# sc15i2gp/daily-ray-trace

Hardware: AMD Instinct MI355X
Metric: Mpaths/s (pixels*spp/s) Cornell 1024^2 depth 8; achieved HBM GB/s % of peak (higher is better)
Workload: dtype f64

## Files before the change

### daily-ray-trace_amd/csrc/drt_kernels.h

```cpp
#pragma once

#include "drt_device.h"
#include "drt_build_rule.h"
#include <type_traits>
#include "../../include/drt_hip.h"


enum
{
    SF_PX = 0, SF_PY, SF_PZ, SF_RADIUS,
    SF_NX, SF_NY, SF_NZ,
    SF_UNX, SF_UNY, SF_UNZ,
    SF_VNX, SF_VNY, SF_VNZ,
    SF_ULEN, SF_VLEN,
    SF_COUNT
};
enum
{
    LF_PX = 0, LF_PY, LF_PZ, LF_RADIUS,
    LF_UX, LF_UY, LF_UZ,
    LF_VX, LF_VY, LF_VZ,
    LF_PDF,
    LF_COUNT
};

enum
{
    NEED_GLOSSY = 1u,
    NEED_EQR    = 2u,
    NEED_EQT    = 4u,
    NEED_CT     = 8u
};

struct BvhNode
{
    float   lo[2][3], hi[2][3];
// ... 877 lines not shown
#define DRT_TRACE_CONST 2
#endif
#if DRT_TRACE_CONST == 1
#define TRACE_CONST_BYTES ((sizeof(TraceConst) + 127u) & ~(size_t)127u)
#else
#define TRACE_CONST_BYTES ((size_t)0)
#endif
__device__ __forceinline__ uint32_t pinned_scalar(uint32_t v)
{
    asm volatile("" : "+s"(v));
    return v;
}
__device__ __forceinline__ const TraceConst &trace_const(const double *lds)
{
#if DRT_TRACE_CONST == 2
    uint32_t off = 0;
    asm volatile("" : "+s"(off));
    return *(const TraceConst *)((const char *)__builtin_amdgcn_kernarg_segment_ptr() + off);
#else
    uint32_t off = 0;
    asm volatile("" : "+v"(off));
    return *(const TraceConst *)((const char *)lds + off);
#endif
}
#define TRACE_LANE_ROWS 2u
#define TRACE_LW_BLK 0u
#define TRACE_LW_DRAWS 1u
#define TRACE_LW_SCANS 128u
#define TRACE_LW_SHADED 129u
__device__ __forceinline__ void lane_word_add(uint32_t *w, uint32_t v)
{
    (void)__hip_atomic_fetch_add(w, v, __ATOMIC_RELAXED, __HIP_MEMORY_SCOPE_WAVEFRONT);
}
#define DRT_TRACE_TAIL_MAX 8u
#ifndef DRT_TRACE_WAVES_PER_SIMD
#define DRT_TRACE_WAVES_PER_SIMD 3
#endif


#ifdef DRT_BRANCH_STATS
#define DRT_BS_WORDS 20
__device__ unsigned long long drt_branch_stats[DRT_BS_WORDS];
__device__ unsigned int drt_branch_waves_done;
#endif

template <bool SCENE_IN_LDS, bool TAIL, bool LIST, bool RAYS>
__device__ __forceinline__ void trace_paths(DevScene k_sc, DevCamera k_cam, TraceParams k_tp,
                                            uint64_t *records, uint64_t *headers,
                                            int32_t *k_hits, unsigned long long *k_counters,
                                            unsigned long long *k_work_counter, const DevRayTable &k_rt)
{
    extern __shared__ double lds_raw[];
#if DRT_TRACE_CONST == 1
    if (threadIdx.x == 0)
    {
        TraceConst *c = (TraceConst *)lds_raw;
        c->sc = k_sc;
        c->cam = k_cam;
        c->tp = k_tp;
        c->hits = k_hits;
        c->counters = k_counters;
        c->work_counter = k_work_counter;
    }
#endif
#if DRT_TRACE_CONST == 0
    const TraceConst k_all = {k_sc, k_cam, k_tp, records, headers, k_hits, k_counters, k_work_counter};
#define LC k_all
#else
#define LC trace_const(lds_raw)
#endif
#if DRT_TRACE_CONST == 2
#define LC_RT (((const TraceRaysConst &)trace_const(lds_raw)).rt)
#else
#define LC_RT k_rt
#endif
    SceneView sv;
    double *l_spd_tail = nullptr, *tail_state = nullptr;
    double *lane_area = nullptr;
    uint32_t *lane_words = nullptr;
    uint32_t TR, max_depth, vertex_words, block_words;
    bool tail_on, record_hits;
    {
    const DevScene &sc = k_sc;
    const TraceParams &tp = k_tp;
    sv.n_surf = sc.n_surf;
    sv.n_lights = sc.n_lights;
    if (SCENE_IN_LDS)
    {
        double *l_rows = lds_raw + TRACE_CONST_BYTES / 8;
        double *l_surf = l_rows + (size_t)SR_STRIDE * sc.n_surf;
        for (uint32_t k = threadIdx.x; k < SR_STRIDE * sc.n_surf; k += TRACE_BLOCK)
        {
            const uint32_t i = k / SR_STRIDE, f = k % SR_STRIDE;
            l_rows[k] = f < SF_COUNT ? sc.surf[f * sc.n_surf + i] : f == SR_TYPE ? __longlong_as_double((long long)sc.surf_type[i]) : 0.0;
        }
        double *l_lights = l_surf + (size_t)SF_COUNT * sc.n_surf;
        uint32_t *l_u32 = (uint32_t *)(l_lights + (size_t)LF_COUNT * sc.n_lights);
        uint32_t n_u32 = 2 * sc.n_surf + 2 * sc.n_lights;
        DevMaterial *l_mats = (DevMaterial *)((char *)l_u32 + (((size_t)n_u32 * 4 + 7) & ~(size_t)7));
        for (uint32_t k = threadIdx.x; k < SF_COUNT * sc.n_surf; k += TRACE_BLOCK) l_surf[k] = sc.surf[k];
        for (uint32_t k = threadIdx.x; k < LF_COUNT * sc.n_lights; k += TRACE_BLOCK) l_lights[k] = sc.lights[k];
        for (uint32_t k = threadIdx.x; k < sc.n_surf; k += TRACE_BLOCK)
        {
            l_u32[k] = sc.surf_type[k];
            l_u32[sc.n_surf + k] = sc.surf_mat[k];
        }
        for (uint32_t k = threadIdx.x; k < sc.n_lights; k += TRACE_BLOCK)
        {
            l_u32[2 * sc.n_surf + k] = sc.light_type[k];
            l_u32[2 * sc.n_surf + sc.n_lights + k] = sc.light_mat[k];
        }
// ... 5 lines not shown
        sv.lights = l_lights;
        sv.surf_type = l_u32;
        sv.surf_mat = l_u32 + sc.n_surf;
        sv.light_type = l_u32 + 2 * sc.n_surf;
        sv.light_mat = l_u32 + 2 * sc.n_surf + sc.n_lights;
        sv.mats = l_mats;
        sv.rows = l_rows;
        sv.bvh_nodes = nullptr;
        sv.bvh_leaf = nullptr;
    }
    else
    {
        sv.surf = sc.surf;
        sv.lights = sc.lights;
        sv.surf_type = sc.surf_type;
        sv.surf_mat = sc.surf_mat;
        sv.light_type = sc.light_type;
        sv.light_mat = sc.light_mat;
        sv.mats = sc.mats;
        sv.bvh_nodes = sc.bvh_nodes;
        sv.bvh_leaf = sc.bvh_leaf;
        __syncthreads();
    }

    TR = tp.tail_count;
    tail_on = TAIL && SCENE_IN_LDS && tp.tail_stage != nullptr;
    lane_area = SCENE_IN_LDS ? (double *)(sv.mats + sc.n_mat) : lds_raw + TRACE_CONST_BYTES / 8;
    if (tail_on)
    {
        l_spd_tail = lane_area;
        for (uint32_t k = threadIdx.x; k < tp.n_spd * TR; k += TRACE_BLOCK) l_spd_tail[k] = tp.spd_tail[k];
        lane_area += (size_t)tp.n_spd * TR;
    }
    lane_area += (size_t)(threadIdx.x >> 6) * ((TRACE_LANE_ROWS + (tail_on ? 1u + 2u * TR : 0u)) * 64u) + (threadIdx.x & 63u);
    lane_words = (uint32_t *)lane_area;
    lane_words[TRACE_LW_BLK] = 0u;
    lane_words[TRACE_LW_DRAWS] = 0u;
    lane_words[TRACE_LW_SCANS] = 0u;
    lane_words[TRACE_LW_SHADED] = 0u;
    if (tail_on)
    {
        tail_state = lane_area + (TRACE_LANE_ROWS + 1u) * 64u;
        __syncthreads();
    }
    max_depth = tp.max_depth;
    vertex_words = tp.vertex_words;
    block_words = tp.block_words;
    record_hits = tp.record_hits != 0u;
    if (*tp.overflow) return;
    }
    bool tail_ok = false;
    const uint32_t lane = threadIdx.x & 63u;
    uint64_t chunk_next = 0, chunk_end = 0;
    PathPos chunk_pos = {0, 0};

    uint32_t w_paths = 0;
#ifdef DRT_BRANCH_STATS
    uint64_t bs[DRT_BS_WORDS] = {};
#endif

    bool alive = false;
    bool exhausted = false;
    uint64_t rs = 1, hit_row = 0;
    uint32_t depth = 0, shaded = 0;
    uint32_t vis0_mask = 0;
    uint32_t plastic_mask = 0;
    V3 ro = v3(0, 0, 0), rd = v3(0, 0, 0);
    uint64_t *hdr = nullptr;
    uint32_t tbl = 0;
    uint32_t spare = ~0u, spare_tbl = ~0u;
    WavePool wp = {0u, 0u, 0u, 0u};

    for (;;)
    {
        unsigned long long idle_mask = __ballot(!alive);
        if (idle_mask != 0ull && !exhausted)
        {
            uint32_t want = (uint32_t)__popcll(idle_mask);
            uint32_t rank = (uint32_t)__popcll(idle_mask & ((1ull << lane) - 1ull));
            uint64_t avail = chunk_end - chunk_next;
            const uint32_t n_samples = LC.tp.n_samples;
            PathPos from = chunk_pos;
            uint32_t ahead = rank;
            if (avail < want)
            {
                if (!alive && rank < avail) alive = true;
                uint32_t taken = (uint32_t)avail;
                const TraceConst &c = LC;
                const uint64_t CHUNK = c.tp.chunk, n_paths_all = c.tp.n_paths;
                unsigned long long base = 0;
                if (lane == 0) base = atomicAdd(c.work_counter, (unsigned long long)CHUNK);
                base = __shfl(base, 0);
                if (base >= n_paths_all)
                {
                    exhausted = true;
                    chunk_next = chunk_end = 0;
                }
                else
                {
                    chunk_next = base;
                    chunk_end = (base + CHUNK < n_paths_all) ? base + CHUNK : n_paths_all;
                    chunk_pos = path_pos_of_id(base, n_samples);
                    uint64_t avail2 = chunk_end - chunk_next;
                    if (!alive && rank >= taken && (uint64_t)(rank - taken) < avail2)
                    {
                        alive = true;
                        from = chunk_pos;
                        ahead = rank - taken;
                    }
                    uint32_t used = (want - taken < avail2) ? (want - taken) : (uint32_t)avail2;
                    chunk_next += used;
                    chunk_pos = path_pos_step(chunk_pos, used, n_samples);
                }
            }
            else
            {
                if (!alive) alive = true;
                chunk_next += want;
                chunk_pos = path_pos_step(chunk_pos, want, n_samples);
            }
            bool started = alive && ((idle_mask >> lane) & 1ull);
            w_paths += (uint32_t)__popcll(__ballot(started));
            if (started)
            {
                const TraceConst &c = LC;
                const PathPos me = path_pos_step(from, ahead, n_samples);
                const uint64_t q = me.q;
                const uint64_t s_local = me.s;
                if (record_hits) hit_row = s_local * c.tp.n_pix + q;
                const uint64_t t = LIST ? (uint64_t)c.tp.pixel_list[q] : q;
                uint32_t i, j;
                tile_pixel_ij(t, c.tp.tile_w, i, j);
                uint32_t x = c.tp.x0 + i;
                uint32_t y = c.tp.y0 + j * c.tp.row_stride;
                uint32_t sample = c.tp.first_sample + (uint32_t)s_local;
                if (LIST) sample += c.tp.sample_base[t];
                uint64_t key = c.tp.seed + (((uint64_t)sample * (uint64_t)c.tp.height + (uint64_t)y) * (uint64_t)c.tp.width + (uint64_t)x);
                rs = drt_splitmix64(key);
                double weight = 1.0;
                if (RAYS) weight = table_ray(LC_RT, c.tp.width, t, x, y, sample, ro, rd);
                else
                {
                    uint32_t drawn = 0;
                    camera_ray(c.cam, c.tp.pixel_scheme, x, y, rs, drawn, ro, rd);
                    lane_word_add(lane_words + TRACE_LW_DRAWS, drawn);
                }
                depth = 0;
                shaded = 0;
                plastic_mask = 0;
                vis0_mask = 0;
                tail_ok = tail_on;
                if (tail_on)
                {
                    const uint32_t tr = pinned_scalar(TR);
#pragma unroll
                    for (uint32_t j = 0; j < DRT_TRACE_TAIL_MAX; j += 1)
                    {
                        if (j >= tr) break;
                        tail_state[(2u * j) * 64u] = 1.0;
                        tail_state[(2u * j + 1u) * 64u] = 0.0;
                    }
                }
                uint64_t slot = q * (uint64_t)c.tp.batch + s_local;
                hdr = headers + slot * REC_HEADER_WORDS;
                const double vignette = (RAYS ? weight : v_dot(rd, c.cam.forward)) * 1.0;
                hdr[1] = (uint64_t)__double_as_longlong(vignette);
                if (tail_on) lane_area[TRACE_LANE_ROWS * 64u] = vignette;
                if (record_hits)
                {
                    int32_t *h = c.hits + ((uint64_t)c.tp.hits_sample_offset * c.tp.n_pix + hit_row) * max_depth;
                    for (uint32_t d = 0; d < max_depth; d += 1) h[d] = -2;
                }
            }
        }
        if (!__any(alive)) break;

        if (!path_spare_block(LC.tp, wp, alive, shaded, spare, spare_tbl, lane))
        {
            hdr[0] = (uint64_t)HDR_TERM_NOT_DONE << 16;
            alive = false;
            lane_word_add(lane_words + TRACE_LW_SCANS, depth);
            lane_word_add(lane_words + TRACE_LW_SHADED, shaded);
        }
        if (alive)
        {
            TraceHit ip;
            find_ray_intersection<SCENE_IN_LDS>(sv, LC.sc, ip, ro, rd DRT_SCAN_STATS_ARG(bs + 16));
            if (record_hits)
            {
                const TraceConst &c = LC;
                c.hits[((uint64_t)c.tp.hits_sample_offset * c.tp.n_pix + hit_row) * max_depth + depth] = ip.index;
            }
            const DevMaterial &mat = sv.mats[ip.surface_mat];
            bool terminal = false;
            uint32_t term = 0, term_spd = 0;
            if (mat.is_black_body && !mat.is_emissive) terminal = true;
            else if (mat.is_black_body && mat.is_emissive)
            {
                terminal = true;
                term = 1;
                term_spd = (uint32_t)mat.emission_spd;
            }
            else
            {
                uint32_t blk = lane_words[TRACE_LW_BLK];
                path_open_vertex(LC.tp, wp, records, shaded, hdr, blk, tbl, spare, spare_tbl);
                lane_words[TRACE_LW_BLK] = blk;
                uint64_t *vrec = records + (uint64_t)blk * block_words + (uint64_t)(shaded & (REC_BLOCK_VERTICES - 1u)) * vertex_words;
// ... 217 lines not shown
                alive = false;
                lane_word_add(lane_words + TRACE_LW_SCANS, depth);
                lane_word_add(lane_words + TRACE_LW_SHADED, shaded);
            }
        }
    }

    uint64_t scans = lane_words[TRACE_LW_SCANS], n_shaded = lane_words[TRACE_LW_SHADED], draws = lane_words[TRACE_LW_DRAWS];
    uint64_t held = (uint64_t)(spare != ~0u) + (uint64_t)(spare_tbl != ~0u);
    for (int off = 32; off > 0; off >>= 1)
    {
        scans += __shfl_down(scans, off);
        n_shaded += __shfl_down(n_shaded, off);
        draws += __shfl_down(draws, off);
        held += __shfl_down(held, off);
    }
    uint64_t vals[6] = {w_paths, scans, n_shaded, n_shaded * sv.n_lights, draws, (uint64_t)wp.handed - held};
    unsigned long long *counters = LC.counters;
    for (int k = 0; k < 6; k += 1)
        if (lane == 0 && vals[k]) atomicAdd(&counters[k], (unsigned long long)vals[k]);
#ifdef DRT_BRANCH_STATS
    for (int k = 0; k < DRT_BS_WORDS; k += 1)
    {
        uint64_t v = bs[k];
        for (int off = 32; off > 0; off >>= 1) v += __shfl_down(v, off);
        if (lane == 0 && v) atomicAdd(&drt_branch_stats[k], (unsigned long long)v);
    }
    __threadfence();
    if (lane == 0 && atomicAdd(&drt_branch_waves_done, 1u) + 1u == gridDim.x * (TRACE_BLOCK / 64u))
    {
        unsigned long long t[DRT_BS_WORDS];
        for (int k = 0; k < DRT_BS_WORDS; k += 1) t[k] = atomicExch(&drt_branch_stats[k], 0ull);
        printf("DRT_BRANCH_STATS iters %llu lanes %llu | disc %llu %llu | ggx %llu %llu | coin %llu %llu | spec %llu %llu | all4 %llu | "
               "loop %llu again %llu | half %llu eqt %llu | uniform %llu | closest plane steps %llu skipped %llu | shadow plane steps %llu skipped %llu\n",
               t[0], t[1], t[2], t[3], t[4], t[5], t[6], t[7], t[8], t[9], t[10], t[11], t[12], t[13], t[14], t[15], t[16], t[17], t[18], t[19]);
        drt_branch_waves_done = 0u;
    }
#endif
#undef LC
#undef LC_RT
}

template <bool SCENE_IN_LDS, bool TAIL = false, bool LIST = false>
__global__ __launch_bounds__(TRACE_BLOCK, DRT_TRACE_WAVES_PER_SIMD) void drt_trace_kernel(DevScene k_sc, DevCamera k_cam, TraceParams k_tp,
                                                                 uint64_t *__restrict__ records, uint64_t *__restrict__ headers,
                                                                 int32_t *__restrict__ k_hits, unsigned long long *__restrict__ k_counters,
                                                                 unsigned long long *__restrict__ k_work_counter)
{
    const DevRayTable no_table = {nullptr, nullptr, nullptr, 0u, 0u, 0u, 0u};
    trace_paths<SCENE_IN_LDS, TAIL, LIST, false>(k_sc, k_cam, k_tp, records, headers, k_hits, k_counters, k_work_counter, no_table);
}

template <bool SCENE_IN_LDS, bool TAIL = false, bool LIST = false>
__global__ __launch_bounds__(TRACE_BLOCK, DRT_TRACE_WAVES_PER_SIMD) void drt_trace_rays_kernel(DevScene k_sc, DevCamera k_cam, TraceParams k_tp,
                                                                 uint64_t *__restrict__ records, uint64_t *__restrict__ headers,
                                                                 int32_t *__restrict__ k_hits, unsigned long long *__restrict__ k_counters,
                                                                 unsigned long long *__restrict__ k_work_counter, DevRayTable k_rt)
{
    trace_paths<SCENE_IN_LDS, TAIL, LIST, true>(k_sc, k_cam, k_tp, records, headers, k_hits, k_counters, k_work_counter, k_rt);
}


#define SHADE_BLOCK 256
#ifndef DRT_SHADE_WAVES_PER_SIMD
#define DRT_SHADE_WAVES_PER_SIMD 4
#endif
#define SHADE_WAVES (SHADE_BLOCK / 64)
#ifndef DRT_SHADE_WAVES_MULTISET
#define DRT_SHADE_WAVES_MULTISET(n) ((n) == 2 ? 3 : 2)
#endif
#define SHADE_WAVES_PER_SIMD_FOR(n) ((n) == 1 ? DRT_SHADE_WAVES_PER_SIMD : DRT_SHADE_WAVES_MULTISET(n))
#ifndef DRT_SHADE_WAVES_SIMPLE
#define DRT_SHADE_WAVES_SIMPLE 5
#endif
#define SHADE_MAX_SETS 4

struct ShadeParams
// ... 1411 lines not shown
```

### daily-ray-trace_amd/csrc/drt_launcher.hip

```cpp
#include "drt_kernels.h"
#include "drt_bvh_kernels.h"
#include "drt_adaptive_kernels.h"
#include "drt_sample_map_kernels.h"
#include "drt_denoise_kernels.h"
#include "drt_feature_kernels.h"
#include "drt_matte_kernels.h"
#include "drt_ray_kernels.h"
#include "drt_update_kernels.h"
#include "drt_build_kernels.h"
#include "drt_material_kernels.h"
#include "drt_depth_kernels.h"
#include "drt_window_kernels.h"
#include "drt_window_rule.h"
#include "drt_owned.h"

#include <algorithm>
#include <cmath>
#include <cstdarg>
#include <cstdio>
#include <cstdlib>
#include <cstring>
#include <map>
#include <string>
#include <chrono>
// ... 74 lines not shown
    DevBuf<double> d_tail_resume;
    uint32_t  batch_spp = 1;
    uint32_t  vertex_words = 0, vertex_shift = 0, block_words = 0;
    uint64_t  pool_blocks = 0;
    uint32_t  worst_blocks_per_path = 0;
    double    est_blocks_per_path = 0.0;
    struct Batch { uint32_t first_sample, n_samples; uint64_t seq; uint32_t row0, rows, hits_sample_offset, stride; const uint32_t *list; uint64_t list_len; };
    std::vector<Batch> inflight;
    uint64_t  next_seq = 1;
    uint64_t  redone_batches = 0, pool_peak = 0;
    DevBuf<int32_t> d_hits;
    uint64_t  hits_capacity = 0;
    uint32_t  hits_samples = 0;
    DevBuf<unsigned long long> d_counters;
    DevBuf<PrimaryHit> d_primary;
    DevBuf<uint64_t> d_queue;
    bool        bvh_pipeline = false;
    int         primary_grid_cap = 0, bounce_grid_cap = 0;
    DevBuf<double> d_xyz;
    DevBuf<uint8_t> d_bgra;
    bool      trace_tail = false;
    bool      tail_all_staged = false;
    bool      tail_resume = false;
    bool      dark_skip = true;
    bool      dark_skip_win = true;
    bool      no_fixed_lists = false;
    bool      simple_bdsfs = false;
    bool      no_closed_shade = false;
    bool      closed_lists = false;
    const double *d_spd_tail = nullptr;

    bool   scene_in_lds = true, spds_in_lds = true, use_bvh = false;
    size_t trace_lds = 0, shade_lds = 0;
    int    trace_grid_cap = 0, shade_grid_cap = 0;
    uint32_t trace_chunk_override = 0, shade_subs_override = ~0u, tail_period_override = 0;
    uint32_t shade_sets = 1, tail_first = 0, tail_count = 0;
    uint64_t n_pix = 0;

    std::vector<Event> ev;
    std::vector<double> ev_paths;
    size_t ev_used = 0;
    double trace_ms = 0.0, shade_ms = 0.0;
    uint64_t timed_pairs = 0;
    double min_sample_ms = 0.0, max_sample_ms = 0.0, avg_sample_ms = 0.0;

    bool film_used = false, adaptive_done = false;
    DevBuf<uint32_t> d_counts;
    DevBuf<uint32_t> d_alist[2];
    DevBuf<unsigned long long> d_keep;
    DevBuf<uint32_t> d_bkeep;
    DevBuf<uint32_t> d_ainfo;
    PinnedBuf<uint32_t> h_active;
    uint64_t film_gen = 0;
    uint64_t dn_gen = 0;
    bool     dn_valid = false;
    DevBuf<double> d_dn_mean, d_dn_var, d_dn_guide, d_dn_weights, d_dn_wsum;
    DevBuf<uint32_t> d_dn_unusable;
    uint32_t dn_window_cap = 0;
    std::vector<drt_material> ft_mats;
    std::vector<double> ft_spds;
    uint32_t ft_n_spd = 0, ft_S = 0;
    DevBuf<double> d_ft_mean, d_ft_m2, d_ft_colour;
    DevBuf<int32_t> d_ft_ids;
    DevBuf<uint32_t> d_ft_counts, d_ft_report;
    DevBuf<unsigned long long> d_ft_info;
    Event    ft_ev[2];
// ... 919 lines not shown
    const uint32_t deepest = (params->max_depth + REC_BLOCK_VERTICES - 1) / REC_BLOCK_VERTICES;
    ctx->worst_blocks_per_path = deepest + (deepest > REC_HEADER_BLOCKS ? 1u : 0u);
    if (deepest > REC_HEADER_BLOCKS + 2 * ctx->block_words)
        return fail(-2, "max_depth %u: a path's table block holds %u blocks beyond the header's %d", params->max_depth, 2 * ctx->block_words, REC_HEADER_BLOCKS);
    if (ctx->dsc.n_spd >= 0xFFFFu) return fail(-2, "too many SPDs for the 16-bit record indices");
    if (S > 64 * SHADE_MAX_SETS) return fail(-2, "more than %d wavelengths", 64 * SHADE_MAX_SETS);
    {
        uint32_t sets = 0, tf = 0, tc = 0;
        shade_sets(S, &sets, &tf, &tc);
        ctx->tail_count = tc;
    }
    ctx->bvh_pipeline = !ctx->scene_in_lds;

    HIP_TRY(ctx->own_pixels.need(pixels_bytes(ctx) / 8));
    if (!ctx->xyz_mode)
    {
        HIP_TRY(ctx->own_avgs.need((size_t)ctx->n_pix * S));
        HIP_TRY(ctx->own_vars.need((size_t)ctx->n_pix * S));
    }
    ctx->d_pixels = ctx->own_pixels;
    ctx->d_avgs = ctx->own_avgs;
    ctx->d_vars = ctx->own_vars;
    ctx->own_film = true;
    HIP_TRY(hipMemsetAsync(ctx->d_pixels, 0, pixels_bytes(ctx), ctx->stream));
    if (ctx->d_avgs) HIP_TRY(hipMemsetAsync(ctx->d_avgs, 0, (size_t)ctx->n_pix * S * 8, ctx->stream));
    if (ctx->d_vars) HIP_TRY(hipMemsetAsync(ctx->d_vars, 0, (size_t)ctx->n_pix * S * 8, ctx->stream));
    HIP_TRY(ctx->d_counters.need(DRT_COUNTER_WORDS));
    HIP_TRY(hipMemsetAsync(ctx->d_counters, 0, DRT_COUNTER_WORDS * sizeof(unsigned long long), ctx->stream));

    hipDeviceProp_t prop;
    HIP_TRY(hipGetDeviceProperties(&prop, ctx->device));
    int per_cu = 0;
    if (ctx->scene_in_lds && ctx->trace_tail)
        HIP_TRY(hipOccupancyMaxActiveBlocksPerMultiprocessor(&per_cu, drt_trace_kernel<true, true>, TRACE_BLOCK, ctx->trace_lds));
    else if (ctx->scene_in_lds)
        HIP_TRY(hipOccupancyMaxActiveBlocksPerMultiprocessor(&per_cu, drt_trace_kernel<true, false>, TRACE_BLOCK, ctx->trace_lds));
    if (per_cu < 1) per_cu = 1;
    if (const char *e = getenv("DRT_TRACE_BLOCKS_PER_CU")) per_cu = std::max(1, atoi(e));
    ctx->trace_grid_cap = prop.multiProcessorCount * per_cu;
    ctx->ray_grid_cap = prop.multiProcessorCount * 4;
    if (const char *e = getenv("DRT_RAY_CHUNK"))
        ctx->ray_chunk = std::max<uint64_t>(1, std::min<uint64_t>(RAY_STAGING_RAYS, strtoull(e, nullptr, 0)));
    if (ctx->bvh_pipeline)
    {
        int p_cu = 0, b_cu = 0;
        HIP_TRY(hipOccupancyMaxActiveBlocksPerMultiprocessor(&p_cu, drt_primary_kernel<false>, PRIMARY_BLOCK, 0));
        HIP_TRY(hipOccupancyMaxActiveBlocksPerMultiprocessor(&b_cu, drt_bounce_kernel<false>, BOUNCE_BLOCK, 0));
        if (const char *e = getenv("DRT_TRACE_BLOCKS_PER_CU")) b_cu = std::max(1, atoi(e));
        ctx->primary_grid_cap = prop.multiProcessorCount * std::max(1, p_cu);
        ctx->bounce_grid_cap = prop.multiProcessorCount * std::max(1, b_cu);
    }
    ctx->shade_lds = ctx->spds_in_lds ? (size_t)ctx->dsc.n_spd * S * 8 : 0;
    ctx->shade_lds += (size_t)SHADE_WAVES * SHADE_WAVE_LDS_WORDS * 8;
    int s_per_cu = 0;
    shade_sets(S, &ctx->shade_sets, &ctx->tail_first, &ctx->tail_count);
    switch (ctx->shade_sets)
    {
        case 1: rc = shade_occupancy<1>(ctx, &s_per_cu); break;
        case 2: rc = shade_occupancy<2>(ctx, &s_per_cu); break;
        case 3: rc = shade_occupancy<3>(ctx, &s_per_cu); break;
        default: rc = shade_occupancy<4>(ctx, &s_per_cu); break;
    }
    if (rc) return rc;
    if (s_per_cu < 1) s_per_cu = 1;
    if (const char *e = getenv("DRT_SHADE_BLOCKS_PER_CU")) s_per_cu = std::max(1, atoi(e));
    ctx->shade_grid_cap = prop.multiProcessorCount * s_per_cu;
    if (const char *e = getenv("DRT_RESERVE_BLOCKS"))
    {
        int n = std::max(0, atoi(e));
// ... 344 lines not shown
    uint32_t grid = (uint32_t)std::min<uint64_t>(blocks_needed, (uint64_t)grid_cap);
    {
        uint64_t waves = (uint64_t)grid * (TRACE_BLOCK / 64);
        uint64_t c = tp.n_paths / (waves * 16) / 64 * 64;
        tp.chunk = (uint32_t)std::min<uint64_t>(std::max<uint64_t>(c, 64), ctx->bvh_pipeline ? 256 : 1024);
        if (ctx->trace_chunk_override) tp.chunk = ctx->trace_chunk_override;
    }
    DevRayTable rt = ctx->rt;
    rt.t_offset = (list || whole) ? 0 : (uint64_t)row0 * p.tile_w;
    const bool rays = ctx->rays_bound;
    if (ctx->bvh_pipeline)
    {
        const uint64_t packets = (tp.n_paths + 63) / 64;
        const uint32_t pgrid = (uint32_t)std::min<uint64_t>((packets + PRIMARY_BLOCK / 64 - 1) / (PRIMARY_BLOCK / 64), (uint64_t)ctx->primary_grid_cap);
#define DRT_BVH_ARGS_P ctx->dsc, ctx->dcam, tp, ctx->d_headers, ctx->d_hits, ctx->d_counters + DRT_PAIR_COUNTERS, ctx->d_primary, ctx->d_queue, work + 2
#define DRT_BVH_ARGS_B ctx->dsc, ctx->dcam, tp, ctx->d_records, ctx->d_headers, ctx->d_hits, ctx->d_counters + DRT_PAIR_COUNTERS, work, ctx->d_primary, ctx->d_queue, work + 2
#define DRT_LAUNCH_BVH(LIST)                                                                                                              \
        if (rays) hipLaunchKernelGGL(drt_primary_rays_kernel<LIST>, dim3(pgrid), dim3(PRIMARY_BLOCK), 0, ctx->stream, DRT_BVH_ARGS_P, rt); \
        else hipLaunchKernelGGL(drt_primary_kernel<LIST>, dim3(pgrid), dim3(PRIMARY_BLOCK), 0, ctx->stream, DRT_BVH_ARGS_P);               \
        HIP_TRY(hipGetLastError());                                                                                                       \
        if (rays) hipLaunchKernelGGL(drt_bounce_rays_kernel<LIST>, dim3(grid), dim3(BOUNCE_BLOCK), 0, ctx->stream, DRT_BVH_ARGS_B, rt);    \
        else hipLaunchKernelGGL(drt_bounce_kernel<LIST>, dim3(grid), dim3(BOUNCE_BLOCK), 0, ctx->stream, DRT_BVH_ARGS_B)
        if (list) { DRT_LAUNCH_BVH(true); }
        else { DRT_LAUNCH_BVH(false); }
#undef DRT_LAUNCH_BVH
#undef DRT_BVH_ARGS_P
#undef DRT_BVH_ARGS_B
    }
    else
    {
#define DRT_TRACE_ARGS ctx->dsc, ctx->dcam, tp, ctx->d_records, ctx->d_headers, ctx->d_hits, ctx->d_counters + DRT_PAIR_COUNTERS, work
#define DRT_LAUNCH_TRACE(TAIL, LIST)                                                                                                                       \
        if (rays) hipLaunchKernelGGL((drt_trace_rays_kernel<true, TAIL, LIST>), dim3(grid), dim3(TRACE_BLOCK), ctx->trace_lds, ctx->stream, DRT_TRACE_ARGS, rt); \
        else hipLaunchKernelGGL((drt_trace_kernel<true, TAIL, LIST>), dim3(grid), dim3(TRACE_BLOCK), ctx->trace_lds, ctx->stream, DRT_TRACE_ARGS)
        const bool tail = ctx->trace_tail && tp.tail_stage;
        if (list && tail) { DRT_LAUNCH_TRACE(true, true); }
        else if (list) { DRT_LAUNCH_TRACE(false, true); }
        else if (tail) { DRT_LAUNCH_TRACE(true, false); }
        else { DRT_LAUNCH_TRACE(false, false); }
#undef DRT_LAUNCH_TRACE
#undef DRT_TRACE_ARGS
    }
    HIP_TRY(hipGetLastError());
    return 0;
}

static int enqueue_pair(drt_context *ctx, uint32_t first_sample, uint32_t n, uint32_t hits_sample_offset, uint32_t row0 = 0, uint32_t rows = 0, uint32_t stride = 0,
                        const uint32_t *list = nullptr, uint64_t list_len = 0)
{
    hipEvent_t ev[3];
    int rc = next_events(ctx, ev);
    if (rc) return rc;
    ctx->film_gen += 1;
    HIP_TRY(hipEventRecord(ev[0], ctx->stream));
    const bool windowed = ctx->win_open && !list;
    const uint32_t t_row0 = rows ? row0 : 0u, t_rows = rows ? rows : ctx->params.tile_h;
    uint32_t l_row0 = t_row0, l_rows = t_rows, l_cols = ctx->params.tile_w;
    if (windowed)
    {
        const uint32_t lo = std::max(t_row0, ctx->wy0), hi = std::min(t_row0 + t_rows, ctx->wy1);
        l_row0 = lo;
        l_rows = hi > lo ? hi - lo : 0u;
        l_cols = ctx->wx1 - ctx->wx0;
    }
    const bool nothing = windowed && (l_rows == 0u || l_cols == 0u);
    if (!windowed && (rc = pool_floor(ctx))) return rc;
    if (windowed) { if (!nothing && (rc = enqueue_trace(ctx, first_sample, n, hits_sample_offset, l_row0, l_rows, stride, nullptr, 0, ctx->wx0, l_cols))) return rc; }
// ... 374 lines not shown
extern "C" int drt_read_hit_indices(drt_context *ctx, int32_t *dst, uint64_t capacity_paths)
{
    if (!ctx || !dst) return fail(-1, "null argument");
    if (!(ctx->params.flags & DRT_FLAG_RECORD_HITS) || !ctx->d_hits) return fail(-4, "hit recording is off (DRT_FLAG_RECORD_HITS)");
    int rc = drt_synchronize(ctx);
    if (rc) return rc;
    uint64_t n = std::min<uint64_t>(capacity_paths, ctx->n_pix * (uint64_t)ctx->hits_samples);
    HIP_TRY(hipMemcpy(dst, ctx->d_hits, n * ctx->params.max_depth * sizeof(int32_t), hipMemcpyDeviceToHost));
    return 0;
}

extern "C" int drt_get_stats(drt_context *ctx, drt_stats *out)
{
    if (!ctx || !out) return fail(-1, "null argument");
    int rc = drt_synchronize(ctx);
    if (rc) return rc;
    unsigned long long c[DRT_NUM_COUNTERS];
    HIP_TRY(hipMemcpy(c, ctx->d_counters, sizeof(c), hipMemcpyDeviceToHost));
    memset(out, 0, sizeof(*out));
    out->paths = c[0];
    out->closest_hit_scans = c[1];
    out->shaded_vertices = c[2];
    out->shadow_scans = c[3];
    out->rng_draws = c[4];
    out->trace_ms = ctx->trace_ms;
    out->shade_ms = ctx->shade_ms;
    out->total_ms = ctx->trace_ms + ctx->shade_ms;
    out->record_pool_blocks = ctx->pool_blocks;
    out->record_pool_peak = ctx->pool_peak;
    out->record_block_bytes = ctx->block_words * 8;
    out->redone_launches = (uint32_t)ctx->redone_batches;
    out->launches = (uint32_t)std::min<uint64_t>(ctx->timed_pairs, 0xFFFFFFFFull);
    out->path_flags = (ctx->bvh_pipeline ? DRT_PATH_BVH : 0u) | ((ctx->trace_tail && ctx->d_tail_stage) ? DRT_PATH_TRACE_TAIL : 0u) |
                      (ctx->rays_bound ? DRT_PATH_RAYS : 0u);
    out->min_sample_ms = ctx->min_sample_ms;
    out->max_sample_ms = ctx->max_sample_ms;
    out->avg_sample_ms = ctx->avg_sample_ms;
    return 0;
}

extern "C" uint32_t drt_batch_spp(drt_context *ctx) { return ctx ? ctx->batch_spp : 0; }

static void window_out(const LiveWindow &w, uint32_t out[4]) { out[0] = w.x_lo; out[1] = w.x_hi; out[2] = w.y_lo; out[3] = w.y_hi; }

extern "C" int drt_live_window_of(const drt_scene *scene, const drt_camera *camera, const drt_params *params, uint32_t out[4])
{
    g_last_error.clear();
    if (!scene || !camera || !params || !out) return fail(-1, "drt_live_window_of: null argument");
    if (scene->escape_material >= scene->num_materials) return fail(-2, "base/escape material index out of range");
    if ((uint64_t)params->x0 + params->tile_w > params->width ||
        (params->tile_h && (uint64_t)params->y0 + (uint64_t)(params->tile_h - 1) * (params->row_stride ? params->row_stride : 1) >= params->height))
        return fail(-1, "tile does not fit the %ux%u image", params->width, params->height);
    drt_params p = *params;
    if (p.row_stride == 0) p.row_stride = 1;
    window_out(live_window_of(scene->surfaces, scene->num_surfaces, scene->materials[scene->escape_material], *camera, p), out);
    return 0;
}

extern "C" int drt_live_window(drt_context *ctx, uint32_t out[4])
{
    if (!ctx || !out) return fail(-1, "drt_live_window: null argument");
    window_refresh(ctx);
    window_out(ctx->win, out);
    return 0;
}

extern "C" int drt_shade_instantiation(const drt_context *ctx)
// ... 3470 lines not shown
```

### daily-ray-trace_amd/pydrt.py

```python
import ctypes as C
import os
import sys

import numpy as np

HERE = os.path.dirname(os.path.abspath(__file__))
REPO = os.path.dirname(HERE)

DRT_MAX_BDSFS = 16
GEO_POINT, GEO_SPHERE, GEO_PLANE = 1, 2, 3
FILM_SAMPLE_CENTER, FILM_SAMPLE_RANDOM = 1, 2
MODE_SPECTRAL, MODE_XYZ = 0, 1
FLAG_RECORD_HITS = 1
BATCH_RESIDENT = 0xFFFFFFFF
FLAG_FILM_ZERO = 2
PATH_BVH, PATH_TRACE_TAIL, PATH_RAYS = 1, 2, 4

BDSF_NAMES = ["bp_diffuse_bdsf", "bp_glossy_bdsf", "mirror_bdsf", "fs_conductor_bdsf",
              "fs_dielectric_reflectance_bdsf", "fs_dielectric_transmittance_bdsf", "ct_conductor_bdsf"]
DIRF_NAMES = ["cos_weighted_sample_hemisphere", "uniform_sample_hemisphere", "sample_specular_direction",
              "sample_transmit_direction", "sample_reflect_or_transmit_direction", "sample_ct_direction"]
BDSF = {n: i for i, n in enumerate(BDSF_NAMES)}
DIRF = {n: i for i, n in enumerate(DIRF_NAMES)}

f64x3 = C.c_double * 3


class Surface(C.Structure):
    _fields_ = [("type", C.c_uint32), ("material", C.c_uint32), ("position", f64x3), ("radius", C.c_double),
                ("normal", f64x3), ("u", f64x3), ("v", f64x3)]


class Material(C.Structure):
    _fields_ = [("is_black_body", C.c_uint32), ("is_emissive", C.c_uint32), ("shininess", C.c_double),
                ("roughness", C.c_double), ("emission_spd", C.c_int32), ("diffuse_spd", C.c_int32),
                ("glossy_spd", C.c_int32), ("mirror_spd", C.c_int32), ("refract_spd", C.c_int32),
                ("extinct_spd", C.c_int32), ("num_bdsfs", C.c_uint32), ("bdsfs", C.c_uint32 * DRT_MAX_BDSFS),
                ("dir_func", C.c_uint32)]


class Scene(C.Structure):
    _fields_ = [("num_surfaces", C.c_uint32), ("surfaces", C.POINTER(Surface)), ("num_materials", C.c_uint32),
                ("materials", C.POINTER(Material)), ("base_material", C.c_uint32), ("escape_material", C.c_uint32),
                ("num_spds", C.c_uint32), ("num_wavelengths", C.c_uint32), ("spds", C.POINTER(C.c_double)),
                ("min_wavelength", C.c_double), ("wavelength_interval", C.c_double), ("cmf_rw", C.c_uint32),
                ("cmf_x", C.c_uint32), ("cmf_y", C.c_uint32), ("cmf_z", C.c_uint32)]


class Camera(C.Structure):
# ... 1383 lines not shown
```

### include/drt_hip.h

```cpp
#ifndef DRT_HIP_H
#define DRT_HIP_H

#include <stdint.h>

#ifdef __cplusplus
extern "C" {
#endif

#define DRT_MAX_BDSFS 16

enum
{
    DRT_GEO_NONE   = 0,
    DRT_GEO_POINT  = 1,
    DRT_GEO_SPHERE = 2,
    DRT_GEO_PLANE  = 3
};

enum
{
    DRT_FILM_SAMPLE_CENTER = 1,
    DRT_FILM_SAMPLE_RANDOM = 2
};

// ... 97 lines not shown
} drt_params;

#define DRT_BATCH_RESIDENT 0xFFFFFFFFu

enum
{
    DRT_FLAG_RECORD_HITS = 1u,
    DRT_FLAG_FILM_ZERO   = 2u
};

typedef struct drt_stats
{
    uint64_t paths;
    uint64_t closest_hit_scans;
    uint64_t shaded_vertices;
    uint64_t shadow_scans;
    uint64_t rng_draws;
    double   trace_ms;
    double   shade_ms;
    double   total_ms;
    uint64_t record_pool_blocks;
    uint64_t record_pool_peak;
    uint32_t record_block_bytes;
    uint32_t redone_launches;
    uint32_t launches;
    uint32_t path_flags;
    double   min_sample_ms, max_sample_ms, avg_sample_ms;
} drt_stats;

enum
{
    DRT_PATH_BVH        = 1u,
    DRT_PATH_TRACE_TAIL = 2u,
    DRT_PATH_RAYS       = 4u
};

typedef struct drt_context drt_context;

const char *drt_last_error(void);
int drt_device_count(void);

drt_context *drt_create(const drt_scene *scene, const drt_camera *camera, const drt_params *params);
void         drt_destroy(drt_context *ctx);
int drt_bind_film(drt_context *ctx, void *d_pixels, void *d_avgs, void *d_vars);
int drt_set_stream(drt_context *ctx, void *hip_stream);
int drt_render(drt_context *ctx, uint32_t first_sample, uint32_t num_samples);
int drt_synchronize(drt_context *ctx);
int drt_reset_film(drt_context *ctx);
int drt_film_device_ptrs(drt_context *ctx, void **d_pixels, void **d_avgs, void **d_vars);
int drt_read_film(drt_context *ctx, double *pixels, double *avgs, double *vars);
int drt_write_film(drt_context *ctx, const double *pixels, const double *avgs, const double *vars);
int drt_read_xyz(drt_context *ctx, double *xyz);
int drt_read_bgra(drt_context *ctx, int which, uint8_t *bgra);
int drt_read_hit_indices(drt_context *ctx, int32_t *dst, uint64_t capacity_paths);
int drt_get_stats(drt_context *ctx, drt_stats *out);
uint32_t drt_batch_spp(drt_context *ctx);

#define DRT_SHADE_GENERAL 0
#define DRT_SHADE_SIMPLE 1
#define DRT_SHADE_CLOSED 2
int drt_shade_instantiation(const drt_context *ctx);

int drt_render_tile(const drt_scene *scene, const drt_camera *camera, const drt_params *params,
                    double *dst_pixels, double *dst_avgs, double *dst_vars, drt_stats *stats);

typedef struct drt_group drt_group;
drt_group *drt_group_create(const drt_scene *scene, const drt_camera *camera, const drt_params *params,
// ... 185 lines not shown
```

Baseline: 2165.

## Stash precomputed camera rays per wave in LDS for path refill

Adds a per-wave LDS stash of up to 64 precomputed camera rays (origin, direction, RNG state, vignette, pixel, sample). When lanes go idle, the whole wave generates a full batch of camera rays at once, and idle lanes pick entries from the stash. Previously only the idle lanes generated rays, so camera-ray generation ran divergent on every refill. The stash costs extra LDS and wave barriers, and the launcher enables it only when occupancy is not reduced and DRT_NO_RAY_STASH is unset.

```diff
diff --git a/daily-ray-trace_amd/csrc/drt_kernels.h b/daily-ray-trace_amd/csrc/drt_kernels.h
--- a/daily-ray-trace_amd/csrc/drt_kernels.h
+++ b/daily-ray-trace_amd/csrc/drt_kernels.h
@@ -2,6 +2,7 @@
 
 #include "drt_device.h"
 #include "drt_build_rule.h"
+#include "drt_stash_rule.h"
 #include <type_traits>
 #include "../../include/drt_hip.h"
 
@@ -945,6 +946,15 @@
 {
     (void)__hip_atomic_fetch_add(w, v, __ATOMIC_RELAXED, __HIP_MEMORY_SCOPE_WAVEFRONT);
 }
+#define TRACE_ST_OX 0u
+#define TRACE_ST_DX 3u
+#define TRACE_ST_RS 6u
+#define TRACE_ST_VIG 7u
+#define TRACE_ST_Q 8u
+#define TRACE_ST_SD 9u
+#define TRACE_STASH_ROWS 10u
+#define TRACE_STASH_WAVE_WORDS (TRACE_STASH_ROWS * 64u + 2u)
+#define TRACE_STASH_BYTES ((size_t)(TRACE_BLOCK / 64) * TRACE_STASH_WAVE_WORDS * 8u)
 #define DRT_TRACE_TAIL_MAX 8u
 #ifndef DRT_TRACE_WAVES_PER_SIMD
 #define DRT_TRACE_WAVES_PER_SIMD 3
@@ -952,13 +962,13 @@
 
 
 #ifdef DRT_BRANCH_STATS
-#define DRT_BS_WORDS 20
+#define DRT_BS_WORDS 23
 __device__ unsigned long long drt_branch_stats[DRT_BS_WORDS];
 __device__ unsigned int drt_branch_waves_done;
 #endif
 
-template <bool SCENE_IN_LDS, bool TAIL, bool LIST, bool RAYS>
-__device__ __forceinline__ void trace_paths(DevScene k_sc, DevCamera k_cam, TraceParams k_tp,
+template <bool SCENE_IN_LDS, bool TAIL, bool LIST, bool RAYS, bool STASH>
+__device__ __forceinline__ void trace_paths_form(DevScene k_sc, DevCamera k_cam, TraceParams k_tp,
                                             uint64_t *records, uint64_t *headers,
                                             int32_t *k_hits, unsigned long long *k_counters,
                                             unsigned long long *k_work_counter, const DevRayTable &k_rt)
@@ -990,6 +1000,7 @@
     SceneView sv;
     double *l_spd_tail = nullptr, *tail_state = nullptr;
     double *lane_area = nullptr;
+    double *stash = nullptr;
     uint32_t *lane_words = nullptr;
     uint32_t TR, max_depth, vertex_words, block_words;
     bool tail_on, record_hits;
@@ -1061,6 +1072,7 @@
         for (uint32_t k = threadIdx.x; k < tp.n_spd * TR; k += TRACE_BLOCK) l_spd_tail[k] = tp.spd_tail[k];
         lane_area += (size_t)tp.n_spd * TR;
     }
+    if (STASH) stash = lane_area + (size_t)(TRACE_BLOCK / 64) * ((TRACE_LANE_ROWS + (tail_on ? 1u + 2u * TR : 0u)) * 64u) + (size_t)(threadIdx.x >> 6) * TRACE_STASH_WAVE_WORDS;
     lane_area += (size_t)(threadIdx.x >> 6) * ((TRACE_LANE_ROWS + (tail_on ? 1u + 2u * TR : 0u)) * 64u) + (threadIdx.x & 63u);
     lane_words = (uint32_t *)lane_area;
     lane_words[TRACE_LW_BLK] = 0u;
@@ -1082,6 +1094,7 @@
     const uint32_t lane = threadIdx.x & 63u;
     uint64_t chunk_next = 0, chunk_end = 0;
     PathPos chunk_pos = {0, 0};
+    StashState st = {0u, 0u};
 
     uint32_t w_paths = 0;
 #ifdef DRT_BRANCH_STATS
@@ -1103,6 +1116,155 @@
     for (;;)
     {
         unsigned long long idle_mask = __ballot(!alive);
+        if constexpr (STASH)
+        {
+        if (idle_mask != 0ull && !exhausted)
+        {
+            const uint32_t want = (uint32_t)__popcll(idle_mask);
+            const uint32_t rank = (uint32_t)__popcll(idle_mask & ((1ull << lane) - 1ull));
+            bool started = false;
+            auto pick = [&](uint32_t entry) __attribute__((always_inline)) {
+                const TraceConst &c = LC;
+                const double *e = stash + entry;
+                ro = v3(e[(TRACE_ST_OX + 0u) * 64u], e[(TRACE_ST_OX + 1u) * 64u], e[(TRACE_ST_OX + 2u) * 64u]);
+                rd = v3(e[(TRACE_ST_DX + 0u) * 64u], e[(TRACE_ST_DX + 1u) * 64u], e[(TRACE_ST_DX + 2u) * 64u]);
+                rs = (uint64_t)__double_as_longlong(e[TRACE_ST_RS * 64u]);
+                const double vignette = e[TRACE_ST_VIG * 64u];
+                const uint64_t q = (uint64_t)__double_as_longlong(e[TRACE_ST_Q * 64u]);
+                const uint64_t sd = (uint64_t)__double_as_longlong(e[TRACE_ST_SD * 64u]);
+                const uint64_t s_local = sd & 0xFFFFFFFFull;
+                lane_word_add(lane_words + TRACE_LW_DRAWS, (uint32_t)(sd >> 32));
+                if (record_hits) hit_row = s_local * c.tp.n_pix + q;
+                const uint64_t slot = q * (uint64_t)c.tp.batch + s_local;
+                hdr = headers + slot * REC_HEADER_WORDS;
+                hdr[1] = (uint64_t)__double_as_longlong(vignette);
+                if (tail_on) lane_area[TRACE_LANE_ROWS * 64u] = vignette;
+                started = true;
+            };
+            const int32_t e1 = stash_first_entry(st, want, rank);
+            if (!alive && e1 >= 0) pick((uint32_t)e1);
+            const uint32_t take1 = stash_after_first(st, want);
+            if (take1 < want)
+            {
+                uint64_t *pos_slot = (uint64_t *)(stash + TRACE_STASH_ROWS * 64u);
+                if (chunk_next == chunk_end)
+                {
+                    const TraceConst &c = LC;
+                    const uint64_t CHUNK = c.tp.chunk, n_paths_all = c.tp.n_paths;
+                    unsigned long long base = 0;
+                    if (lane == 0) base = atomicAdd(c.work_counter, (unsigned long long)CHUNK);
+                    base = (unsigned long long)(uint32_t)__builtin_amdgcn_readfirstlane((int)(uint32_t)base) |
+                           ((unsigned long long)(uint32_t)__builtin_amdgcn_readfirstlane((int)(uint32_t)(base >> 32)) << 32);
+                    if (base >= n_paths_all)
+                    {
+                        exhausted = true;
+                        chunk_next = chunk_end = 0;
+                    }
+                    else
+                    {
+                        chunk_next = base;
+                        chunk_end = (base + CHUNK < n_paths_all) ? base + CHUNK : n_paths_all;
+                        const PathPos p0 = path_pos_of_id(base, c.tp.n_samples);
+                        if (lane == 0)
+                        {
+                            pos_slot[0] = p0.q;
+                            pos_slot[1] = (uint64_t)p0.s;
+                        }
+                        __builtin_amdgcn_fence(__ATOMIC_SEQ_CST, "wavefront");
+                        __builtin_amdgcn_wave_barrier();
+                    }
+                }
+                if (!exhausted)
+                {
+                    const uint32_t n = stash_fill_size(chunk_next, chunk_end);
+                    PathPos from;
+                    from.q = pos_slot[0];
+                    from.s = (uint32_t)pos_slot[1];
+                    const uint32_t n_samples = LC.tp.n_samples;
+                    if (lane < n)
+                    {
+                        const TraceConst &c = LC;
+                        const PathPos me = path_pos_step(from, lane, n_samples);
+                        const uint64_t q = me.q;
+                        const uint64_t s_local = me.s;
+                        const uint64_t t = LIST ? (uint64_t)c.tp.pixel_list[q] : q;
+                        uint32_t i, j;
+                        tile_pixel_ij(t, c.tp.tile_w, i, j);
+                        const uint32_t x = c.tp.x0 + i;
+                        const uint32_t y = c.tp.y0 + j * c.tp.row_stride;
+                        uint32_t sample = c.tp.first_sample + (uint32_t)s_local;
+                        if (LIST) sample += c.tp.sample_base[t];
+                        const uint64_t key = c.tp.seed + (((uint64_t)sample * (uint64_t)c.tp.height + (uint64_t)y) * (uint64_t)c.tp.width + (uint64_t)x);
+                        uint64_t f_rs = drt_splitmix64(key);
+                        uint32_t drawn = 0;
+                        V3 f_ro, f_rd;
+                        camera_ray(c.cam, c.tp.pixel_scheme, x, y, f_rs, drawn, f_ro, f_rd);
+                        const double vignette = v_dot(f_rd, c.cam.forward) * 1.0;
+                        double *w = stash + lane;
+                        w[(TRACE_ST_OX + 0u) * 64u] = f_ro.x;
+                        w[(TRACE_ST_OX + 1u) * 64u] = f_ro.y;
+                        w[(TRACE_ST_OX + 2u) * 64u] = f_ro.z;
+                        w[(TRACE_ST_DX + 0u) * 64u] = f_rd.x;
+                        w[(TRACE_ST_DX + 1u) * 64u] = f_rd.y;
+                        w[(TRACE_ST_DX + 2u) * 64u] = f_rd.z;
+                        w[TRACE_ST_RS * 64u] = __longlong_as_double((long long)f_rs);
+                        w[TRACE_ST_VIG * 64u] = vignette;
+                        w[TRACE_ST_Q * 64u] = __longlong_as_double((long long)q);
+                        w[TRACE_ST_SD * 64u] = __longlong_as_double((long long)(s_local | ((uint64_t)drawn << 32)));
+                    }
+                    if (lane == 0)
+                    {
+                        const PathPos next = path_pos_step(from, n, n_samples);
+                        pos_slot[0] = next.q;
+                        pos_slot[1] = (uint64_t)next.s;
+                    }
+                    __builtin_amdgcn_fence(__ATOMIC_SEQ_CST, "wavefront");
+                    __builtin_amdgcn_wave_barrier();
+                    const int32_t e2 = stash_second_entry(n, want, take1, rank);
+                    if (!alive && !started && e2 >= 0) pick((uint32_t)e2);
+                    stash_after_fill(st, chunk_next, n, want, take1);
+                }
+            }
+            w_paths += (uint32_t)__popcll(__ballot(started));
+#ifdef DRT_BRANCH_STATS
+            {
+                const unsigned long long m_started = __ballot(started);
+                if (m_started != 0ull && lane == 0u)
+                {
+                    bs[20] += 1;
+                    bs[21] += __popcll(m_started);
+                }
+            }
+#endif
+            if (started)
+            {
+                alive = true;
+                depth = 0;
+                shaded = 0;
+                plastic_mask = 0;
+                vis0_mask = 0;
+                tail_ok = tail_on;
+                if (tail_on)
+                {
+                    const uint32_t tr = pinned_scalar(TR);
+#pragma unroll
+                    for (uint32_t j = 0; j < DRT_TRACE_TAIL_MAX; j += 1)
+                    {
+                        if (j >= tr) break;
+                        tail_state[(2u * j) * 64u] = 1.0;
+                        tail_state[(2u * j + 1u) * 64u] = 0.0;
+                    }
+                }
+                if (record_hits)
+                {
+                    const TraceConst &c = LC;
+                    int32_t *h = c.hits + ((uint64_t)c.tp.hits_sample_offset * c.tp.n_pix + hit_row) * max_depth;
+                    for (uint32_t d = 0; d < max_depth; d += 1) h[d] = -2;
+                }
+            }
+        }
+        }
+        else
         if (idle_mask != 0ull && !exhausted)
         {
             uint32_t want = (uint32_t)__popcll(idle_mask);
@@ -1150,6 +1312,16 @@
             }
             bool started = alive && ((idle_mask >> lane) & 1ull);
             w_paths += (uint32_t)__popcll(__ballot(started));
+#ifdef DRT_BRANCH_STATS
+            {
+                const unsigned long long m_started = __ballot(started);
+                if (m_started != 0ull && lane == 0u)
+                {
+                    bs[20] += 1;
+                    bs[21] += __popcll(m_started);
+                }
+            }
+#endif
             if (started)
             {
                 const TraceConst &c = LC;
@@ -1203,6 +1375,9 @@
             }
         }
         if (!__any(alive)) break;
+#ifdef DRT_BRANCH_STATS
+        if (lane == 0u) bs[22] += 1;
+#endif
 
         if (!path_spare_block(LC.tp, wp, alive, shaded, spare, spare_tbl, lane))
         {
@@ -1486,8 +1661,10 @@
         unsigned long long t[DRT_BS_WORDS];
         for (int k = 0; k < DRT_BS_WORDS; k += 1) t[k] = atomicExch(&drt_branch_stats[k], 0ull);
         printf("DRT_BRANCH_STATS iters %llu lanes %llu | disc %llu %llu | ggx %llu %llu | coin %llu %llu | spec %llu %llu | all4 %llu | "
-               "loop %llu again %llu | half %llu eqt %llu | uniform %llu | closest plane steps %llu skipped %llu | shadow plane steps %llu skipped %llu\n",
-               t[0], t[1], t[2], t[3], t[4], t[5], t[6], t[7], t[8], t[9], t[10], t[11], t[12], t[13], t[14], t[15], t[16], t[17], t[18], t[19]);
+               "loop %llu again %llu | half %llu eqt %llu | uniform %llu | closest plane steps %llu skipped %llu | shadow plane steps %llu skipped %llu | "
+               "starts entered %llu lanes %llu of %llu wave-iterations\n",
+               t[0], t[1], t[2], t[3], t[4], t[5], t[6], t[7], t[8], t[9], t[10], t[11], t[12], t[13], t[14], t[15], t[16], t[17], t[18], t[19],
+               t[20], t[21], t[22]);
         drt_branch_waves_done = 0u;
     }
 #endif
@@ -1495,8 +1672,27 @@
 #undef LC_RT
 }
 
+template <bool SCENE_IN_LDS, bool TAIL, bool LIST, bool RAYS>
+__device__ __forceinline__ void trace_paths(DevScene k_sc, DevCamera k_cam, TraceParams k_tp,
+                                            uint64_t *records, uint64_t *headers,
+                                            int32_t *k_hits, unsigned long long *k_counters,
+                                            unsigned long long *k_work_counter, const DevRayTable &k_rt)
+{
+    trace_paths_form<SCENE_IN_LDS, TAIL, LIST, RAYS, false>(k_sc, k_cam, k_tp, records, headers, k_hits, k_counters, k_work_counter, k_rt);
+}
+
 template <bool SCENE_IN_LDS, bool TAIL = false, bool LIST = false>
 __global__ __launch_bounds__(TRACE_BLOCK, DRT_TRACE_WAVES_PER_SIMD) void drt_trace_kernel(DevScene k_sc, DevCamera k_cam, TraceParams k_tp,
+                                                                 uint64_t *__restrict__ records, uint64_t *__restrict__ headers,
+                                                                 int32_t *__restrict__ k_hits, unsigned long long *__restrict__ k_counters,
+                                                                 unsigned long long *__restrict__ k_work_counter)
+{
+    const DevRayTable no_table = {nullptr, nullptr, nullptr, 0u, 0u, 0u, 0u};
+    trace_paths_form<SCENE_IN_LDS, TAIL, LIST, false, SCENE_IN_LDS>(k_sc, k_cam, k_tp, records, headers, k_hits, k_counters, k_work_counter, no_table);
+}
+
+template <bool SCENE_IN_LDS, bool TAIL = false, bool LIST = false>
+__global__ __launch_bounds__(TRACE_BLOCK, DRT_TRACE_WAVES_PER_SIMD) void drt_trace_direct_kernel(DevScene k_sc, DevCamera k_cam, TraceParams k_tp,
                                                                  uint64_t *__restrict__ records, uint64_t *__restrict__ headers,
                                                                  int32_t *__restrict__ k_hits, unsigned long long *__restrict__ k_counters,
                                                                  unsigned long long *__restrict__ k_work_counter)
diff --git a/daily-ray-trace_amd/csrc/drt_launcher.hip b/daily-ray-trace_amd/csrc/drt_launcher.hip
--- a/daily-ray-trace_amd/csrc/drt_launcher.hip
+++ b/daily-ray-trace_amd/csrc/drt_launcher.hip
@@ -130,6 +130,7 @@
 
     bool   scene_in_lds = true, spds_in_lds = true, use_bvh = false;
     size_t trace_lds = 0, shade_lds = 0;
+    bool trace_stash = false;
     int    trace_grid_cap = 0, shade_grid_cap = 0;
     uint32_t trace_chunk_override = 0, shade_subs_override = ~0u, tail_period_override = 0;
     uint32_t shade_sets = 1, tail_first = 0, tail_count = 0;
@@ -1115,9 +1116,17 @@
     HIP_TRY(hipGetDeviceProperties(&prop, ctx->device));
     int per_cu = 0;
     if (ctx->scene_in_lds && ctx->trace_tail)
-        HIP_TRY(hipOccupancyMaxActiveBlocksPerMultiprocessor(&per_cu, drt_trace_kernel<true, true>, TRACE_BLOCK, ctx->trace_lds));
+        HIP_TRY(hipOccupancyMaxActiveBlocksPerMultiprocessor(&per_cu, drt_trace_direct_kernel<true, true>, TRACE_BLOCK, ctx->trace_lds));
     else if (ctx->scene_in_lds)
-        HIP_TRY(hipOccupancyMaxActiveBlocksPerMultiprocessor(&per_cu, drt_trace_kernel<true, false>, TRACE_BLOCK, ctx->trace_lds));
+        HIP_TRY(hipOccupancyMaxActiveBlocksPerMultiprocessor(&per_cu, drt_trace_direct_kernel<true, false>, TRACE_BLOCK, ctx->trace_lds));
+    ctx->trace_stash = false;
+    if (ctx->scene_in_lds && !(getenv("DRT_NO_RAY_STASH") && atoi(getenv("DRT_NO_RAY_STASH")) != 0) && ctx->trace_lds + TRACE_STASH_BYTES <= 64 * 1024)
+    {
+        int with = 0;
+        if (ctx->trace_tail) HIP_TRY(hipOccupancyMaxActiveBlocksPerMultiprocessor(&with, drt_trace_kernel<true, true>, TRACE_BLOCK, ctx->trace_lds + TRACE_STASH_BYTES));
+        else HIP_TRY(hipOccupancyMaxActiveBlocksPerMultiprocessor(&with, drt_trace_kernel<true, false>, TRACE_BLOCK, ctx->trace_lds + TRACE_STASH_BYTES));
+        ctx->trace_stash = with >= 1 && with >= per_cu;
+    }
     if (per_cu < 1) per_cu = 1;
     if (const char *e = getenv("DRT_TRACE_BLOCKS_PER_CU")) per_cu = std::max(1, atoi(e));
     ctx->trace_grid_cap = prop.multiProcessorCount * per_cu;
@@ -1528,7 +1537,8 @@
 #define DRT_TRACE_ARGS ctx->dsc, ctx->dcam, tp, ctx->d_records, ctx->d_headers, ctx->d_hits, ctx->d_counters + DRT_PAIR_COUNTERS, work
 #define DRT_LAUNCH_TRACE(TAIL, LIST)                                                                                                                       \
         if (rays) hipLaunchKernelGGL((drt_trace_rays_kernel<true, TAIL, LIST>), dim3(grid), dim3(TRACE_BLOCK), ctx->trace_lds, ctx->stream, DRT_TRACE_ARGS, rt); \
-        else hipLaunchKernelGGL((drt_trace_kernel<true, TAIL, LIST>), dim3(grid), dim3(TRACE_BLOCK), ctx->trace_lds, ctx->stream, DRT_TRACE_ARGS)
+        else if (ctx->trace_stash) hipLaunchKernelGGL((drt_trace_kernel<true, TAIL, LIST>), dim3(grid), dim3(TRACE_BLOCK), ctx->trace_lds + TRACE_STASH_BYTES, ctx->stream, DRT_TRACE_ARGS); \
+        else hipLaunchKernelGGL((drt_trace_direct_kernel<true, TAIL, LIST>), dim3(grid), dim3(TRACE_BLOCK), ctx->trace_lds, ctx->stream, DRT_TRACE_ARGS)
         const bool tail = ctx->trace_tail && tp.tail_stage;
         if (list && tail) { DRT_LAUNCH_TRACE(true, true); }
         else if (list) { DRT_LAUNCH_TRACE(false, true); }
@@ -1969,7 +1979,7 @@
     out->redone_launches = (uint32_t)ctx->redone_batches;
     out->launches = (uint32_t)std::min<uint64_t>(ctx->timed_pairs, 0xFFFFFFFFull);
     out->path_flags = (ctx->bvh_pipeline ? DRT_PATH_BVH : 0u) | ((ctx->trace_tail && ctx->d_tail_stage) ? DRT_PATH_TRACE_TAIL : 0u) |
-                      (ctx->rays_bound ? DRT_PATH_RAYS : 0u);
+                      (ctx->rays_bound ? DRT_PATH_RAYS : 0u) | ((ctx->trace_stash && !ctx->bvh_pipeline) ? DRT_PATH_RAY_STASH : 0u);
     out->min_sample_ms = ctx->min_sample_ms;
     out->max_sample_ms = ctx->max_sample_ms;
     out->avg_sample_ms = ctx->avg_sample_ms;
diff --git a/daily-ray-trace_amd/csrc/drt_stash_rule.h b/daily-ray-trace_amd/csrc/drt_stash_rule.h
--- /dev/null
+++ b/daily-ray-trace_amd/csrc/drt_stash_rule.h
@@ -0,0 +1,51 @@
+#ifndef DRT_STASH_RULE_H
+#define DRT_STASH_RULE_H
+
+#include <cstdint>
+
+#if defined(__HIPCC__) || defined(__CUDACC__)
+#define DRT_STASH_FN __host__ __device__ __forceinline__
+#else
+#define DRT_STASH_FN static inline
+#endif
+
+#define DRT_STASH_ENTRIES 64u
+
+struct StashState
+{
+    uint32_t head;
+    uint32_t count;
+};
+
+DRT_STASH_FN uint32_t stash_take(uint32_t want, uint32_t have) { return want < have ? want : have; }
+
+DRT_STASH_FN uint32_t stash_fill_size(uint64_t chunk_next, uint64_t chunk_end)
+{
+    const uint64_t rest = chunk_end - chunk_next;
+    return rest < (uint64_t)DRT_STASH_ENTRIES ? (uint32_t)rest : DRT_STASH_ENTRIES;
+}
+
+DRT_STASH_FN int32_t stash_first_entry(const StashState &st, uint32_t want, uint32_t rank)
+{
+    return rank < stash_take(want, st.count) ? (int32_t)(st.head + rank) : -1;
+}
+DRT_STASH_FN uint32_t stash_after_first(StashState &st, uint32_t want)
+{
+    const uint32_t take1 = stash_take(want, st.count);
+    st.head += take1;
+    st.count -= take1;
+    return take1;
+}
+DRT_STASH_FN int32_t stash_second_entry(uint32_t n, uint32_t want, uint32_t take1, uint32_t rank)
+{
+    return (rank >= take1 && rank - take1 < stash_take(want - take1, n)) ? (int32_t)(rank - take1) : -1;
+}
+DRT_STASH_FN void stash_after_fill(StashState &st, uint64_t &chunk_next, uint32_t n, uint32_t want, uint32_t take1)
+{
+    const uint32_t take2 = stash_take(want - take1, n);
+    st.head = take2;
+    st.count = n - take2;
+    chunk_next += n;
+}
+
+#endif
diff --git a/daily-ray-trace_amd/pydrt.py b/daily-ray-trace_amd/pydrt.py
--- a/daily-ray-trace_amd/pydrt.py
+++ b/daily-ray-trace_amd/pydrt.py
@@ -14,7 +14,7 @@
 FLAG_RECORD_HITS = 1
 BATCH_RESIDENT = 0xFFFFFFFF
 FLAG_FILM_ZERO = 2
-PATH_BVH, PATH_TRACE_TAIL, PATH_RAYS = 1, 2, 4
+PATH_BVH, PATH_TRACE_TAIL, PATH_RAYS, PATH_RAY_STASH = 1, 2, 4, 8
 
 BDSF_NAMES = ["bp_diffuse_bdsf", "bp_glossy_bdsf", "mirror_bdsf", "fs_conductor_bdsf",
               "fs_dielectric_reflectance_bdsf", "fs_dielectric_transmittance_bdsf", "ct_conductor_bdsf"]
diff --git a/include/drt_hip.h b/include/drt_hip.h
--- a/include/drt_hip.h
+++ b/include/drt_hip.h
@@ -153,7 +153,8 @@
 {
     DRT_PATH_BVH        = 1u,
     DRT_PATH_TRACE_TAIL = 2u,
-    DRT_PATH_RAYS       = 4u
+    DRT_PATH_RAYS       = 4u,
+    DRT_PATH_RAY_STASH  = 8u
 };
 
 typedef struct drt_context drt_context;
```

After: 2211 (median of 6 runs). 2.1% higher.
